# cyberlife-coder/velesdb

Hardware: AMD Instinct MI355X
Metric: qps_at_recall10_1Mx768_k10 (higher is better)
Workload: dtype f32; 1 GPU; 1000000x768 f32 cosine, k=10, exact distance sweep + fused GPU top-k (BASELINE configs[1]); 1024 queries/step, 1024 queries per corpus pass (sweep_topk_gemm_bf16_pp<dot, WIDE> over normalised bf16 images of rows and queries (cosine; ping-po; rows=1000000, dim=768, k=10, parallelism=replicas x1 (query stream split, no collective)

## Files before the change

velesdb_amd/csrc/sweep_wide.hip:

```cpp
#include <algorithm>

#include "vdb_device.hpp"
#include "vdb_kernels.hpp"
#include "vdb_wide.hpp"
#include "vdb_block_select.hpp"

namespace vdb {

__device__ __forceinline__ float wide_eps(uint32_t dim, const float* rho_q, const uint32_t* rho_max_bits, uint32_t q, float extra = 0.0f) {
  const float acc = 16.0f * (float)dim * 5.9604645e-8f;
  if (!rho_q || !rho_max_bits) return 2.0f * 3.90625e-3f * 1.002f + 1.6e-5f + acc + extra;
  const float rm = __uint_as_float(*rho_max_bits), rq = rho_q[q];
  return (rm + rq + 3.0f * rm * rq) * 1.002f + acc + 4e-6f + extra;
}

__device__ __forceinline__ uint64_t wide_tau_key(float s_k, float delta, bool* ok, float extra = 0.0f) {
  const float lowered = s_k - 2.0f * delta * 1.01f - extra - fabsf(s_k) * 1e-6f;
  *ok = lowered == lowered && fabsf(lowered) < 3.0e38f;
  return make_key<true>(lowered, 0u);
}
__device__ __forceinline__ uint64_t wide_tau_closed() { return make_key<true>(3.0e38f, 0u); }

template <int METRIC>
__global__ __launch_bounds__(256) void wide_seed_kernel(WideArgs a, const uint64_t* seed_keys, uint32_t ngrp) {
  __shared__ uint32_t hist[256];
  __shared__ uint32_t ctl[2];
  const uint32_t q = blockIdx.x, tid = threadIdx.x;
  constexpr int NPT = kWideSeedGroups / 256;
  uint64_t keys[NPT];
  uint32_t mine = 0;
#pragma unroll
  for (int j = 0; j < NPT; j++) {
    const uint32_t i = tid + 256u * (uint32_t)j;
    keys[j] = i < ngrp ? seed_keys[(size_t)q * ngrp + i] : kKeyInvalid;
    mine += keys[j] != kKeyInvalid ? 1u : 0u;
  }
  const float eps = wide_eps(a.dim, a.rho_q, a.rho_max_bits, q, a.eps_extra);
  const float d = METRIC == kCosine ? eps * 1.001f + 4e-7f : eps * 1.001f * a.qnorms[q] * __uint_as_float(*a.norm_max_bits) + 1e-30f;
  __shared__ uint32_t total;
  if (tid == 0) total = 0;
  __syncthreads();
  if (mine) atomicAdd(&total, mine);
  __syncthreads();
  const uint32_t valid = total;
  bool ok = valid >= a.k && d == d;
  uint64_t tau = wide_tau_closed();
  if (ok) {
    __shared__ uint64_t s256[256];
    const uint32_t hi = ngrp <= 256 ? block_kth_hi_256(keys[0], a.k, s256, ctl) : block_kth_hi<NPT>(keys, a.k, hist, ctl);
    tau = wide_tau_key(key_score<true>((uint64_t)hi << 32), d, &ok);
    if (!ok) tau = wide_tau_closed();
  }
  if (tid == 0) {
    a.delta[q] = d;
    a.tau[q] = tau;
    a.cnt[q] = 0;
    a.state[q] = ok ? 0u : kWideGivenUp;
  }
}

template <int NPT>
__device__ int wide_next_tau(const WideArgs& a, uint32_t raw, const uint64_t (&keys)[NPT], float delta, float extra, uint64_t old, uint32_t* hist,
                             uint32_t* ctl, uint64_t* s256, uint64_t* tau_out) {
  if (raw > a.cap) return 2;
  if (raw < a.k) return 0;
  const uint32_t hi = raw <= 256 ? block_kth_hi_256(keys[0], a.k, s256, ctl, (raw + 7u) & ~7u) : block_kth_hi<NPT>(keys, a.k, hist, ctl);
  bool ok;
  uint64_t tau = wide_tau_key(key_score<true>((uint64_t)hi << 32), delta, &ok, extra);
  if (!ok) return 2;
  if (tau > old) tau = old;
  *tau_out = tau;
  return 1;
}

__global__ __launch_bounds__(256) void wide_reseed_kernel(WideArgs a) {
  __shared__ uint32_t hist[256];
  __shared__ uint32_t ctl[2];
  __shared__ uint32_t wsum[4];
  __shared__ uint64_t s256[256];
  const uint32_t q = blockIdx.x, tid = threadIdx.x;
  const uint32_t state = a.state[q], raw = a.cnt[q];
  const float delta = a.delta[q], extra = a.extra ? a.extra[q] : 0.0f;
  const uint64_t old = a.tau[q];
  if (state & kWideGivenUp) return;
  constexpr int NPT = kWideCap / 256;
  uint64_t* list = a.keys + (size_t)q * a.cap;
  uint64_t keys[NPT];
  keys[0] = list[tid];
  if (tid >= raw) keys[0] = kKeyInvalid;
#pragma unroll
  for (int j = 1; j < NPT; j++) {
    const uint32_t i = tid + 256u * (uint32_t)j;
    keys[j] = (i < raw && i < a.cap) ? list[i] : kKeyInvalid;
  }
  uint64_t tau = 0;
  const int what = wide_next_tau<NPT>(a, raw, keys, delta, extra, old, hist, ctl, s256, &tau);
  if (what == 0) return;
  if (what == 2) {
    if (tid == 0) {
      a.state[q] |= kWideGivenUp;
      a.tau[q] = wide_tau_closed();
    }
    return;
  }
  uint32_t keep = 0;
#pragma unroll
  for (int j = 0; j < NPT; j++) keep += (keys[j] != kKeyInvalid && keys[j] < tau) ? 1u : 0u;
  uint32_t incl = keep;
  const uint32_t lane = tid & 63u, w = tid >> 6;
#pragma unroll
  for (int o = 1; o < 64; o <<= 1) {
    const uint32_t up = __shfl_up(incl, o, 64);
    if ((int)lane >= o) incl += up;
  }
  if (lane == 63) wsum[w] = incl;
  __syncthreads();
  uint32_t base = incl - keep;
  for (uint32_t x = 0; x < w; x++) base += wsum[x];
#pragma unroll
  for (int j = 0; j < NPT; j++)
    if (keys[j] != kKeyInvalid && keys[j] < tau) list[base++] = keys[j];
  if (tid == 0) {
    a.cnt[q] = wsum[0] + wsum[1] + wsum[2] + wsum[3];
    a.tau[q] = tau;
  }
}

template <int METRIC>
__global__ __launch_bounds__(256) void wide_rerank_verify(WideArgs a, WideOutArgs o, bool fuse) {
  extern __shared__ __attribute__((aligned(16))) unsigned char smem[];
  constexpr uint32_t kStep = 64, kStride = kStep + 4, kChunk = 64;
  float* qs = reinterpret_cast<float*>(smem);
  uint64_t* ekeys = reinterpret_cast<uint64_t*>(qs + o.dim_pad);
  float* stage = reinterpret_cast<float*>(ekeys + kWidePoolMax);
  uint32_t* crow = reinterpret_cast<uint32_t*>(stage + 2 * kChunk * kStride);
  uint64_t* kth = reinterpret_cast<uint64_t*>(crow + kChunk);
  __shared__ uint32_t cand[kWidePoolMax];
  __shared__ uint32_t hist[256];
  __shared__ uint32_t ctl[2];
  __shared__ uint32_t wsum[4];
  __shared__ uint64_t s256[256];
  const uint32_t tid = threadIdx.x, qi = blockIdx.x;
  auto stamp = [&](int i) {
    if (o.stamps && tid == 0) o.stamps[(size_t)qi * 8 + i] = wall_clock64();
  };
  stamp(0);
  const float* q = o.queries + (size_t)qi * o.q_stride;
  const uint64_t* list = a.keys + (size_t)qi * a.cap;
  float qreg[4];
#pragma unroll
  for (int j = 0; j < 4; j++) {
    const uint32_t i = tid + 256u * (uint32_t)j;
    qreg[j] = i < a.dim ? q[i] : 0.0f;
  }
  const uint64_t first = list[tid];
  const float qn = METRIC == kCosine ? a.qnorms[qi] : 0.0f;
  const uint32_t raw = a.cnt[qi];
  bool given_up = (a.state[qi] & kWideGivenUp) != 0 || raw > a.cap;
  uint64_t tau_fin = a.tau[qi];
  const float delta = a.delta[qi], extra = a.extra ? a.extra[qi] : 0.0f;
  uint32_t n = 0;
  if (fuse) {
    constexpr int NPT = kWideCap / 256;
    uint64_t keys[NPT];
    keys[0] = (!given_up && tid < raw) ? first : kKeyInvalid;
#pragma unroll
    for (int j = 1; j < NPT; j++) {
      const uint32_t i = tid + 256u * (uint32_t)j;
      keys[j] = (!given_up && i < raw) ? list[i] : kKeyInvalid;
    }
    if (!given_up) {
      uint64_t t = 0;
      const int what = wide_next_tau<NPT>(a, raw, keys, delta, extra, tau_fin, hist, ctl, s256, &t);
      if (what == 2) given_up = true;
      if (what == 1) tau_fin = t;
    }
    uint32_t keep = 0;
#pragma unroll
    for (int j = 0; j < NPT; j++) keep += (keys[j] != kKeyInvalid && keys[j] < tau_fin) ? 1u : 0u;
    uint32_t incl = keep;
    const uint32_t lane = tid & 63u, w = tid >> 6;
#pragma unroll
    for (int s = 1; s < 64; s <<= 1) {
      const uint32_t up = __shfl_up(incl, s, 64);
      if ((int)lane >= s) incl += up;
    }
    if (lane == 63) wsum[w] = incl;
    __syncthreads();
    uint32_t base = incl - keep;
    for (uint32_t x = 0; x < w; x++) base += wsum[x];
    const uint32_t total = wsum[0] + wsum[1] + wsum[2] + wsum[3];
    if (total > kWidePoolMax) given_up = true;
    if (!given_up) {
      n = total;
#pragma unroll
      for (int j = 0; j < NPT; j++)
        if (keys[j] != kKeyInvalid && keys[j] < tau_fin) cand[base++] = key_row(keys[j]);
    }
  } else {
    if (raw > kWidePoolMax) given_up = true;
    n = given_up ? 0u : raw;
    if (tid < n) cand[tid] = key_row(first);
    for (uint32_t i = tid + 256; i < n; i += 256) cand[i] = key_row(list[i]);
  }
  stamp(1);
#pragma unroll
  for (int j = 0; j < 4; j++) {
    const uint32_t i = tid + 256u * (uint32_t)j;
    if (i < o.dim_pad) qs[i] = qreg[j];
  }
  for (uint32_t i = tid + 1024; i < o.dim_pad; i += 256) qs[i] = i < a.dim ? q[i] : 0.0f;
  if (tid == 0) *kth = kKeyInvalid;
  for (uint32_t c0 = 0; c0 < n; c0 += kChunk) {
    const uint32_t nc = min(kChunk, n - c0);
    __syncthreads();
    if (tid < nc) crow[tid] = cand[c0 + tid];
    __syncthreads();
    uint32_t sh = 0;
    while (sh < 3 && (nc << (sh + 1)) <= kChunk) sh++;
    const uint32_t W = kStep << sh, rowf4 = (kStep / 4) << sh, wstride = W + 4;
    const uint32_t nf4 = nc * rowf4;
    float4 vr[4][4];
    auto fetch = [&](float4 (&v)[4], uint32_t U) {
#pragma unroll
      for (int i = 0; i < 4; i++) {
        const uint32_t f = tid + 256u * (uint32_t)i;
        const uint32_t r = f >> (4 + sh), c4 = f & (rowf4 - 1);
        v[i] = (f < nf4 && U + 4 * c4 < a.dim) ? ld4(o.rows + (size_t)crow[r] * o.row_stride + U + 4 * c4) : make_float4(0.0f, 0.0f, 0.0f, 0.0f);
      }
    };
    auto park = [&](const float4 (&v)[4], uint32_t buf) {
#pragma unroll
      for (int i = 0; i < 4; i++) {
        const uint32_t f = tid + 256u * (uint32_t)i;
        const uint32_t r = f >> (4 + sh), c4 = f & (rowf4 - 1);
        if (f < nf4) *reinterpret_cast<float4*>(stage + (size_t)buf * kChunk * kStride + (size_t)r * wstride + 4 * c4) = v[i];
      }
    };
    float acc = 0.0f;
    auto chain = [&](uint32_t U, uint32_t buf) {
      if (tid < nc) {
        const float* x = stage + (size_t)buf * kChunk * kStride + (size_t)tid * wstride;
        const uint32_t groups = min(W, o.dim_pad - U) / 16;
#pragma unroll 4
        for (uint32_t m = 0; m < groups; m++) {
          float xr[16];
#pragma unroll
          for (int e = 0; e < 16; e += 4) {
            const float4 w = *reinterpret_cast<const float4*>(x + 16 * m + e);
            xr[e] = w.x; xr[e + 1] = w.y; xr[e + 2] = w.z; xr[e + 3] = w.w;
          }
          const uint32_t base = U + 16 * m;
#pragma unroll
          for (int c = 0; c < 4; c++)
#pragma unroll
            for (int kk = 0; kk < 4; kk++) acc = __builtin_fmaf(xr[4 * kk + c], qs[base + 4 * kk + c], acc);
        }
      }
    };
    const uint32_t nsteps = (o.dim_pad + W - 1) / W;
    fetch(vr[0], 0);
    if (1 < nsteps) fetch(vr[1], W);
    if (2 < nsteps) fetch(vr[2], 2 * W);
    const float vnorm = (METRIC == kCosine && tid < nc) ? o.norms[crow[tid]] : 1.0f;
    park(vr[0], 0);
    __syncthreads();
    if (c0 == 0) stamp(2);
    for (uint32_t s0 = 0; s0 < nsteps; s0 += 4) {
#pragma unroll
      for (int j = 0; j < 4; j++) {
        const uint32_t st = s0 + (uint32_t)j;
        if (st < nsteps) {
          if (st + 3 < nsteps) fetch(vr[(j + 3) & 3], (st + 3) * W);
          chain(st * W, st & 1u);
          if (st + 1 < nsteps) park(vr[(j + 1) & 3], (st + 1) & 1u);
          __syncthreads();
        }
      }
    }
    if (c0 == 0) stamp(3);
    if (tid < nc) {
      const uint32_t row = crow[tid];
      const float score = finish_score<METRIC>(acc, qn, vnorm);
      ekeys[c0 + tid] = make_key<true>(score, row);
    }
  }
  __syncthreads();
  stamp(4);
  const uint32_t kk = min(a.k, n);
  for (uint32_t i = tid; i < n; i += 256) {
    const uint64_t key = ekeys[i];
    uint32_t rank = 0;
    for (uint32_t j = 0; j < n; j++) rank += ekeys[j] < key ? 1u : 0u;
    if (rank < kk) {
      const uint32_t row = key_row(key);
      o.out_ids[(size_t)qi * a.k + rank] = o.ext_ids ? o.ext_ids[row] : (uint64_t)row;
      o.out_scores[(size_t)qi * a.k + rank] = key_score<true>(key);
      if (rank + 1 == a.k) *kth = key;
    }
  }
  for (uint32_t e = kk + tid; e < a.k; e += 256) {
    o.out_ids[(size_t)qi * a.k + e] = ~0ull;
    o.out_scores[(size_t)qi * a.k + e] = __uint_as_float(0x7FC00000u);
  }
  __syncthreads();
  stamp(5);
  if (tid == 0) {
    bool ok = !given_up && n >= a.k;
    if (ok) {
      const float A = key_score<true>(tau_fin);
      const double Ek = (double)key_score<true>(*kth);
      ok = Ek > (double)A + (double)delta;
    }
    if (fuse) a.tau[qi] = tau_fin;
    o.flags[qi] = ok ? 0u : 1u;
    if (!ok) {
      const uint32_t j = atomicAdd(o.qcount, 1u);
      o.qmap[j] = qi;
      o.qslot[qi] = j;
    }
    o.out_n[qi] = kk;
    if (o.stamps) {
      o.stamps[(size_t)qi * 8 + 6] = wall_clock64();
      o.stamps[(size_t)qi * 8 + 7] = ((unsigned long long)raw << 32) | n;
    }
  }
}

__global__ __launch_bounds__(256) void wide_seed_l2_kernel(WideArgs a, const uint64_t* seed_keys, uint32_t ngrp, uint32_t dim_a) {
  __shared__ uint32_t hist[256];
  __shared__ uint32_t ctl[2];
  __shared__ uint32_t total;
  const uint32_t q = blockIdx.x, tid = threadIdx.x;
  constexpr int NPT = kWideSeedGroups / 256;
  uint64_t keys[NPT];
  uint32_t mine = 0;
#pragma unroll
  for (int j = 0; j < NPT; j++) {
    const uint32_t i = tid + 256u * (uint32_t)j;
    keys[j] = i < ngrp ? seed_keys[(size_t)q * ngrp + i] : kKeyInvalid;
    mine += keys[j] != kKeyInvalid ? 1u : 0u;
  }
  if (tid == 0) total = 0;
  __syncthreads();
  if (mine) atomicAdd(&total, mine);
  __syncthreads();
  const uint32_t valid = total;
  const float nmax = __uint_as_float(*a.norm_max_bits), hmax = 0.5f * nmax * nmax, qn = a.qnorms[q];
  const float acc = 16.0f * (float)dim_a * 5.9604645e-8f;
  float eps_r = 2.0f * 3.90625e-3f * 1.002f + 1.6e-5f + acc;
  if (a.rho_q && a.rho_max_bits) {
    const float rm = __uint_as_float(*a.rho_max_bits), rq = a.rho_q[q];
    eps_r = (rm + rq + 3.0f * rm * rq) * 1.002f + acc;
  }
  const float d = eps_r * 1.001f * qn * nmax + (1.6e-5f + acc) * hmax + 1e-30f;
  const float slack = 8.0f * (float)a.dim * 5.9604645e-8f * (qn * qn + nmax * nmax) * 1.01f + 1e-30f;
  bool ok = valid >= a.k && d == d && slack == slack;
  uint64_t tau = wide_tau_closed();
  if (ok) {
    const uint32_t hi = block_kth_hi<NPT>(keys, a.k, hist, ctl);
    tau = wide_tau_key(key_score<true>((uint64_t)hi << 32), d, &ok, slack);
    if (!ok) tau = wide_tau_closed();
  }
  if (tid == 0) {
    a.delta[q] = d;
    a.extra[q] = slack;
    a.tau[q] = tau;
    a.cnt[q] = 0;
    a.state[q] = ok ? 0u : kWideGivenUp;
  }
}

__global__ __launch_bounds__(256) void wide_rerank_l2(WideArgs a, WideOutArgs o) {
  __shared__ uint64_t ekeys[kWidePoolMax];
  __shared__ float esums[kWidePoolMax];
  __shared__ float kth_sum;
  const int lane = lane_id();
  const uint32_t wib = threadIdx.x >> 6, tid = threadIdx.x, qi = blockIdx.x;
  const uint32_t raw = a.cnt[qi];
  const bool given_up = (a.state[qi] & kWideGivenUp) != 0 || raw > kWidePoolMax || raw > a.cap;
  const uint32_t n = given_up ? 0u : raw;
  const float* q = o.queries + (size_t)qi * o.q_stride;
  const uint64_t* list = a.keys + (size_t)qi * a.cap;
  const int d4 = (int)((a.dim + 3) / 4);
  if (tid == 0) kth_sum = __uint_as_float(0x7FC00000u);
  for (uint32_t c0 = wib; c0 < n; c0 += 16) {
    const float* p[4];
    uint32_t rowv[4];
    float acc[4] = {0.0f, 0.0f, 0.0f, 0.0f};
#pragma unroll
    for (int u = 0; u < 4; u++) {
      const uint32_t c = min(c0 + 4u * (uint32_t)u, n - 1u);
      rowv[u] = key_row(list[c]);
      p[u] = o.rows + (size_t)rowv[u] * o.row_stride;
    }
    for (int ch = lane; ch < d4; ch += 64) {
      const int nv = (int)a.dim - ch * 4;
      float4 x[4];
#pragma unroll
      for (int u = 0; u < 4; u++) x[u] = ld4(p[u] + ch * 4);
      float4 qq;
      if (nv >= 4) {
        qq = make_float4(q[ch * 4], q[ch * 4 + 1], q[ch * 4 + 2], q[ch * 4 + 3]);
#pragma unroll
        for (int u = 0; u < 4; u++) acc[u] = chain4<kOpL2>(acc[u], qq, x[u]);
      } else {
        qq = make_float4(q[ch * 4], nv > 1 ? q[ch * 4 + 1] : 0.f, nv > 2 ? q[ch * 4 + 2] : 0.f, 0.f);
#pragma unroll
        for (int u = 0; u < 4; u++) acc[u] = chain4_tail<kOpL2>(acc[u], qq, x[u], nv);
      }
    }
#pragma unroll
    for (int u = 0; u < 4; u++) {
      const uint32_t c = c0 + 4u * (uint32_t)u;
      const float sum = butterfly_all(acc[u]);
      if (lane == 0 && c < n) {
        esums[c] = sum;
        ekeys[c] = make_key<false>(finish_score<kEuclidean>(sum, 0.f, 0.f), rowv[u]);
      }
    }
  }
  __syncthreads();
  const uint32_t kk = min(a.k, n);
  for (uint32_t i = tid; i < n; i += 256) {
    const uint64_t key = ekeys[i];
    uint32_t rank = 0;
    for (uint32_t j = 0; j < n; j++) rank += ekeys[j] < key ? 1u : 0u;
    if (rank < kk) {
      const uint32_t row = key_row(key);
      o.out_ids[(size_t)qi * a.k + rank] = o.ext_ids ? o.ext_ids[row] : (uint64_t)row;
      o.out_scores[(size_t)qi * a.k + rank] = key_score<false>(key);
      if (rank + 1 == a.k) kth_sum = esums[i];
    }
  }
  for (uint32_t e = kk + tid; e < a.k; e += 256) {
    o.out_ids[(size_t)qi * a.k + e] = ~0ull;
    o.out_scores[(size_t)qi * a.k + e] = __uint_as_float(0x7FC00000u);
  }
  __syncthreads();
  if (tid == 0) {
    bool ok = !given_up && n >= a.k;
    if (ok) {
      const double A = (double)key_score<true>(a.tau[qi]);
      const double qn = (double)a.qnorms[qi];
      const double Ek = (double)kth_sum;
      ok = (Ek + (double)a.extra[qi] + 1e-6 * Ek) < qn * qn - 2.0 * (A + (double)a.delta[qi]);
    }
    o.flags[qi] = ok ? 0u : 1u;
    if (!ok) {
      const uint32_t j = atomicAdd(o.qcount, 1u);
      o.qmap[j] = qi;
      o.qslot[qi] = j;
    }
    o.out_n[qi] = kk;
  }
}

template <int METRIC>
__global__ __launch_bounds__(256) void wide_rerank_sq8(WideArgs a, WideOutArgs o) {
  extern __shared__ __attribute__((aligned(16))) unsigned char smem[];
  float* qs = reinterpret_cast<float*>(smem);
  uint64_t* ekeys = reinterpret_cast<uint64_t*>(qs + ((a.dim + 3) & ~3u));
  float* qred = reinterpret_cast<float*>(ekeys + kWidePoolMax);
  uint64_t* kth = reinterpret_cast<uint64_t*>(qred + 2);
  const uint32_t tid = threadIdx.x, qi = blockIdx.x;
  const uint32_t raw = a.cnt[qi];
  const bool given_up = (a.state[qi] & kWideGivenUp) != 0 || raw > kWidePoolMax || raw > a.cap;
  const uint32_t n = given_up ? 0u : raw;
  const float* q = o.queries + (size_t)qi * o.q_stride;
  for (uint32_t i = tid; i < a.dim; i += 256) qs[i] = q[i];
  if (tid == 0) *kth = kKeyInvalid;
  __syncthreads();
  if (tid == 64) {
    float s1 = 0.0f;
    for (uint32_t d = 0; d < a.dim; d++) s1 = __fadd_rn(s1, qs[d]);
    qred[0] = s1;
  }
  if (tid == 128) {
    float s2 = 0.0f;
    for (uint32_t d = 0; d < a.dim; d++) s2 = __fadd_rn(s2, __fmul_rn(qs[d], qs[d]));
    qred[1] = s2;
  }
  __syncthreads();
  const uint64_t* list = a.keys + (size_t)qi * a.cap;
  for (uint32_t c = tid; c < n; c += 256) {
    const uint32_t row = key_row(list[c]);
    const float mn = o.sq8_min[row], range = __fsub_rn(o.sq8_max[row], mn);
    const uint32_t* cw = reinterpret_cast<const uint32_t*>(o.sq8_codes + (size_t)row * o.sq8_stride);
    float acc = 0.0f;
    if (range < 1.1920929e-07f) {
      acc = __fmul_rn(qred[0], mn);
    } else {
      const float scale = __fdiv_rn(range, 255.0f);
      for (uint32_t i = 0; i < a.dim; i += 4) {
        const uint32_t w = cw[i >> 2];
#pragma unroll
        for (int e = 0; e < 4; e++)
          if (i + e < a.dim) {
            const float dq = __fadd_rn(__fmul_rn((float)((w >> (8 * e)) & 0xFFu), scale), mn);
            acc = __fadd_rn(acc, __fmul_rn(qs[i + e], dq));
          }
      }
    }
    float score = acc;
    if (METRIC == kCosine) {
      const float denom = sqrtf(__fmul_rn(qred[1], o.sq8_nsq[row]));
      score = denom < 1.1920929e-07f ? 0.0f : __fdiv_rn(acc, denom);
    }
    ekeys[c] = make_key<true>(score, row);
  }
  __syncthreads();
  const uint32_t kk = min(a.k, n);
  for (uint32_t i = tid; i < n; i += 256) {
    const uint64_t key = ekeys[i];
    uint32_t rank = 0;
    for (uint32_t j = 0; j < n; j++) rank += ekeys[j] < key ? 1u : 0u;
    if (rank < kk) {
      const uint32_t row = key_row(key);
      o.out_ids[(size_t)qi * a.k + rank] = o.ext_ids ? o.ext_ids[row] : (uint64_t)row;
      o.out_scores[(size_t)qi * a.k + rank] = key_score<true>(key);
      if (rank + 1 == a.k) *kth = key;
    }
  }
  for (uint32_t e = kk + tid; e < a.k; e += 256) {
    o.out_ids[(size_t)qi * a.k + e] = ~0ull;
    o.out_scores[(size_t)qi * a.k + e] = __uint_as_float(0x7FC00000u);
  }
  __syncthreads();
  if (tid == 0) {
    bool ok = !given_up && n >= a.k;
    if (ok) {
      const float A = key_score<true>(a.tau[qi]);
      const double Ek = (double)key_score<true>(*kth);
      ok = Ek > (double)A + (double)a.delta[qi];
    }
    o.flags[qi] = ok ? 0u : 1u;
    if (!ok) {
      const uint32_t j = atomicAdd(o.qcount, 1u);
      o.qmap[j] = qi;
      o.qslot[qi] = j;
    }
    o.out_n[qi] = kk;
  }
}

void launch_wide_seed(int metric, const WideArgs& a, const uint64_t* seed_keys, uint32_t ngrp, uint32_t nq, hipStream_t st) {
  if (metric == kCosine)
    hipLaunchKernelGGL((wide_seed_kernel<kCosine>), dim3(nq), dim3(256), 0, st, a, seed_keys, ngrp);
  else
    hipLaunchKernelGGL((wide_seed_kernel<kDot>), dim3(nq), dim3(256), 0, st, a, seed_keys, ngrp);
}
void launch_wide_reseed(const WideArgs& a, uint32_t nq, hipStream_t st) { hipLaunchKernelGGL(wide_reseed_kernel, dim3(nq), dim3(256), 0, st, a); }
void launch_wide_seed_l2(const WideArgs& a, const uint64_t* seed_keys, uint32_t ngrp, uint32_t dim_a, uint32_t nq, hipStream_t st) {
  hipLaunchKernelGGL(wide_seed_l2_kernel, dim3(nq), dim3(256), 0, st, a, seed_keys, ngrp, dim_a);
}
void launch_wide_rerank_l2(const WideArgs& a, const WideOutArgs& o, uint32_t nq, hipStream_t st) {
  hipLaunchKernelGGL(wide_rerank_l2, dim3(nq), dim3(256), 0, st, a, o);
}
void launch_wide_rerank_sq8(int metric, const WideArgs& a, const WideOutArgs& o, uint32_t nq, hipStream_t st) {
  const size_t lds = ((size_t)((a.dim + 3) & ~3u) * 4 + (size_t)kWidePoolMax * 8 + 8 + 8 + 15) & ~(size_t)15;
  if (metric == kCosine)
    hipLaunchKernelGGL((wide_rerank_sq8<kCosine>), dim3(nq), dim3(256), lds, st, a, o);
  else
    hipLaunchKernelGGL((wide_rerank_sq8<kDot>), dim3(nq), dim3(256), lds, st, a, o);
}
size_t wide_rerank_lds_bytes(uint32_t dim_pad) {
  return ((size_t)dim_pad * 4 + (size_t)kWidePoolMax * 8 + 2 * (size_t)64 * 68 * 4 + 64 * 4 + 8 + 15) & ~(size_t)15;
}
void launch_wide_rerank(int metric, const WideArgs& a, const WideOutArgs& o, uint32_t nq, bool fuse_final_reseed, hipStream_t st) {
  const size_t lds = wide_rerank_lds_bytes(o.dim_pad);
  if (metric == kCosine)
    hipLaunchKernelGGL((wide_rerank_verify<kCosine>), dim3(nq), dim3(256), lds, st, a, o, fuse_final_reseed);
  else
    hipLaunchKernelGGL((wide_rerank_verify<kDot>), dim3(nq), dim3(256), lds, st, a, o, fuse_final_reseed);
}

}
```

Before: 788,800 queries/s.

## Alias rerank LDS regions by phase and read query via scalar loads

Rewrites the rerank-verify kernel's shared-memory plan so candidate ids, exact keys, the staging buffer and selection scratch alias each other by phase. This shrinks LDS, and launch bounds now request 4 blocks per SIMD. The query vector stays in LDS only when it fits next to the candidate pool; otherwise it is read through constant-address-space (scalar) loads in a hand-scheduled, double-buffered FMA loop. Staging rows drop padding and use an XOR swizzle against bank conflicts, and per-query scalars are made wave-uniform with readfirstlane. This risks aliasing hazards between phases (cand is interleaved inside ekeys) and adds complexity, all to raise occupancy and cut LDS traffic in the rerank stage.

```diff
diff --git a/velesdb_amd/csrc/sweep_wide.hip b/velesdb_amd/csrc/sweep_wide.hip
--- a/velesdb_amd/csrc/sweep_wide.hip
+++ b/velesdb_amd/csrc/sweep_wide.hip
@@ -3,6 +3,7 @@
 #include "vdb_device.hpp"
 #include "vdb_kernels.hpp"
 #include "vdb_wide.hpp"
+#include "vdb_wide_rerank_plan.hpp"
 #include "vdb_block_select.hpp"
 
 namespace vdb {
@@ -126,39 +127,45 @@
   }
 }
 
+typedef const __attribute__((address_space(4))) float* wide_cfloat_ptr;
+
 template <int METRIC>
-__global__ __launch_bounds__(256) void wide_rerank_verify(WideArgs a, WideOutArgs o, bool fuse) {
+__global__ __launch_bounds__(256, 4) void wide_rerank_verify(WideArgs a, WideOutArgs o, bool fuse) {
   extern __shared__ __attribute__((aligned(16))) unsigned char smem[];
-  constexpr uint32_t kStep = 64, kStride = kStep + 4, kChunk = 64;
-  float* qs = reinterpret_cast<float*>(smem);
-  uint64_t* ekeys = reinterpret_cast<uint64_t*>(qs + o.dim_pad);
-  float* stage = reinterpret_cast<float*>(ekeys + kWidePoolMax);
-  uint32_t* crow = reinterpret_cast<uint32_t*>(stage + 2 * kChunk * kStride);
-  uint64_t* kth = reinterpret_cast<uint64_t*>(crow + kChunk);
-  __shared__ uint32_t cand[kWidePoolMax];
-  __shared__ uint32_t hist[256];
-  __shared__ uint32_t ctl[2];
-  __shared__ uint32_t wsum[4];
-  __shared__ uint64_t s256[256];
+  constexpr uint32_t kStep = kWideRerankStep, kChunk = kWideRerankChunk, kBuf = kWideRerankBufFloats;
+  static_assert(kWideRerankPool == kWidePoolMax, "vdb_wide_rerank_plan.hpp restates it");
+  const WideRerankPlan lp = wide_rerank_plan(o.dim_pad, a.k);
+  uint64_t* ekeys = reinterpret_cast<uint64_t*>(smem + lp.ekeys.off);
+  uint32_t* cand = reinterpret_cast<uint32_t*>(ekeys);
+  float* stage = reinterpret_cast<float*>(smem + lp.stage.off);
+  uint64_t* s256 = reinterpret_cast<uint64_t*>(smem + lp.s256.off);
+  uint32_t* hist = reinterpret_cast<uint32_t*>(smem + lp.hist.off);
+  uint32_t* ctl = reinterpret_cast<uint32_t*>(smem + lp.ctl.off);
+  uint32_t* wsum = reinterpret_cast<uint32_t*>(smem + lp.wsum.off);
+  uint64_t* kth = reinterpret_cast<uint64_t*>(smem + lp.kth.off);
   const uint32_t tid = threadIdx.x, qi = blockIdx.x;
   auto stamp = [&](int i) {
     if (o.stamps && tid == 0) o.stamps[(size_t)qi * 8 + i] = wall_clock64();
   };
   stamp(0);
   const float* q = o.queries + (size_t)qi * o.q_stride;
-  const uint64_t* list = a.keys + (size_t)qi * a.cap;
   float qreg[4];
 #pragma unroll
   for (int j = 0; j < 4; j++) {
     const uint32_t i = tid + 256u * (uint32_t)j;
     qreg[j] = i < a.dim ? q[i] : 0.0f;
   }
+  const wide_cfloat_ptr qc = (wide_cfloat_ptr)q;
+  const uint64_t* list = a.keys + (size_t)qi * a.cap;
   const uint64_t first = list[tid];
-  const float qn = METRIC == kCosine ? a.qnorms[qi] : 0.0f;
-  const uint32_t raw = a.cnt[qi];
-  bool given_up = (a.state[qi] & kWideGivenUp) != 0 || raw > a.cap;
-  uint64_t tau_fin = a.tau[qi];
-  const float delta = a.delta[qi], extra = a.extra ? a.extra[qi] : 0.0f;
+  auto uni = [](uint32_t v) { return (uint32_t)__builtin_amdgcn_readfirstlane((int)v); };
+  auto unif = [&](float v) { return __uint_as_float(uni(__float_as_uint(v))); };
+  auto uni64 = [&](uint64_t v) { return ((uint64_t)uni((uint32_t)(v >> 32)) << 32) | uni((uint32_t)v); };
+  const float qn = METRIC == kCosine ? unif(a.qnorms[qi]) : 0.0f;
+  const uint32_t raw = uni(a.cnt[qi]);
+  bool given_up = (uni(a.state[qi]) & kWideGivenUp) != 0 || raw > a.cap;
+  uint64_t tau_fin = uni64(a.tau[qi]);
+  const float delta = unif(a.delta[qi]), extra = a.extra ? unif(a.extra[qi]) : 0.0f;
   uint32_t n = 0;
   if (fuse) {
     constexpr int NPT = kWideCap / 256;
@@ -195,38 +202,44 @@
       n = total;
 #pragma unroll
       for (int j = 0; j < NPT; j++)
-        if (keys[j] != kKeyInvalid && keys[j] < tau_fin) cand[base++] = key_row(keys[j]);
+        if (keys[j] != kKeyInvalid && keys[j] < tau_fin) cand[2 * base++] = key_row(keys[j]);
     }
   } else {
     if (raw > kWidePoolMax) given_up = true;
     n = given_up ? 0u : raw;
-    if (tid < n) cand[tid] = key_row(first);
-    for (uint32_t i = tid + 256; i < n; i += 256) cand[i] = key_row(list[i]);
-  }
+    if (tid < n) cand[2 * tid] = key_row(first);
+    for (uint32_t i = tid + 256; i < n; i += 256) cand[2 * i] = key_row(list[i]);
+  }
+  n = uni(n);
+  tau_fin = uni64(tau_fin);
+  given_up = uni(given_up ? 1u : 0u) != 0;
   stamp(1);
-#pragma unroll
-  for (int j = 0; j < 4; j++) {
-    const uint32_t i = tid + 256u * (uint32_t)j;
-    if (i < o.dim_pad) qs[i] = qreg[j];
-  }
-  for (uint32_t i = tid + 1024; i < o.dim_pad; i += 256) qs[i] = i < a.dim ? q[i] : 0.0f;
-  if (tid == 0) *kth = kKeyInvalid;
+  const bool q_lds = wide_rerank_query_in_lds(o.dim_pad, n);
+  const float* qs = reinterpret_cast<const float*>(smem + lp.ekeys.off + wide_rerank_query_off(o.dim_pad));
+  if (q_lds) {
+    float* qw = const_cast<float*>(qs);
+#pragma unroll
+    for (int j = 0; j < 4; j++) {
+      const uint32_t i = tid + 256u * (uint32_t)j;
+      if (i < o.dim_pad) qw[i] = qreg[j];
+    }
+    for (uint32_t i = tid + 1024; i < o.dim_pad; i += 256) qw[i] = i < a.dim ? q[i] : 0.0f;
+  }
+  __syncthreads();
   for (uint32_t c0 = 0; c0 < n; c0 += kChunk) {
     const uint32_t nc = min(kChunk, n - c0);
-    __syncthreads();
-    if (tid < nc) crow[tid] = cand[c0 + tid];
-    __syncthreads();
+    const uint32_t* crow = cand + 2 * c0;
     uint32_t sh = 0;
     while (sh < 3 && (nc << (sh + 1)) <= kChunk) sh++;
-    const uint32_t W = kStep << sh, rowf4 = (kStep / 4) << sh, wstride = W + 4;
+    const uint32_t W = kStep << sh, rowf4 = (kStep / 4) << sh;
     const uint32_t nf4 = nc * rowf4;
     float4 vr[4][4];
-    auto fetch = [&](float4 (&v)[4], uint32_t U) {
+    auto fetch = [&](float4 (&v)[4], uint32_t U, bool on) {
 #pragma unroll
       for (int i = 0; i < 4; i++) {
         const uint32_t f = tid + 256u * (uint32_t)i;
         const uint32_t r = f >> (4 + sh), c4 = f & (rowf4 - 1);
-        v[i] = (f < nf4 && U + 4 * c4 < a.dim) ? ld4(o.rows + (size_t)crow[r] * o.row_stride + U + 4 * c4) : make_float4(0.0f, 0.0f, 0.0f, 0.0f);
+        v[i] = (on && f < nf4 && U + 4 * c4 < a.dim) ? ld4(o.rows + (size_t)crow[2 * r] * o.row_stride + U + 4 * c4) : make_float4(0.0f, 0.0f, 0.0f, 0.0f);
       }
     };
     auto park = [&](const float4 (&v)[4], uint32_t buf) {
@@ -234,35 +247,85 @@
       for (int i = 0; i < 4; i++) {
         const uint32_t f = tid + 256u * (uint32_t)i;
         const uint32_t r = f >> (4 + sh), c4 = f & (rowf4 - 1);
-        if (f < nf4) *reinterpret_cast<float4*>(stage + (size_t)buf * kChunk * kStride + (size_t)r * wstride + 4 * c4) = v[i];
+        if (f < nf4) *reinterpret_cast<float4*>(stage + (size_t)buf * kBuf + (size_t)r * W + 4 * (c4 ^ (r & (rowf4 - 1)))) = v[i];
       }
     };
     float acc = 0.0f;
-    auto chain = [&](uint32_t U, uint32_t buf) {
+    auto load_x = [&](float4 (&x)[4], const float* xrow, uint32_t sw, uint32_t m) {
+#pragma unroll
+      for (int e = 0; e < 4; e++) x[e] = *reinterpret_cast<const float4*>(xrow + 4 * ((4 * m + (uint32_t)e) ^ sw));
+    };
+    auto load_q = [&](float (&qv)[16], uint32_t base) {
+      const wide_cfloat_ptr p = qc + base;
+#pragma unroll
+      for (int e = 0; e < 16; e++) qv[e] = p[e];
+    };
+    auto load_q_tail = [&](float (&qv)[16], uint32_t base) {
+      const wide_cfloat_ptr p = qc + base;
+#pragma unroll
+      for (int e = 0; e < 16; e++) qv[e] = base + e < a.dim ? p[e] : 0.0f;
+    };
+    auto fma16 = [&](const float4 (&x)[4], const float (&qv)[16]) {
+      const float xr[16] = {x[0].x, x[0].y, x[0].z, x[0].w, x[1].x, x[1].y, x[1].z, x[1].w,
+                            x[2].x, x[2].y, x[2].z, x[2].w, x[3].x, x[3].y, x[3].z, x[3].w};
+#pragma unroll
+      for (int c = 0; c < 4; c++)
+#pragma unroll
+        for (int kk = 0; kk < 4; kk++) acc = __builtin_fmaf(xr[4 * kk + c], qv[4 * kk + c], acc);
+    };
+    auto chain = [&](uint32_t U_v, uint32_t buf) {
       if (tid < nc) {
-        const float* x = stage + (size_t)buf * kChunk * kStride + (size_t)tid * wstride;
-        const uint32_t groups = min(W, o.dim_pad - U) / 16;
-#pragma unroll 4
-        for (uint32_t m = 0; m < groups; m++) {
-          float xr[16];
-#pragma unroll
-          for (int e = 0; e < 16; e += 4) {
-            const float4 w = *reinterpret_cast<const float4*>(x + 16 * m + e);
-            xr[e] = w.x; xr[e + 1] = w.y; xr[e + 2] = w.z; xr[e + 3] = w.w;
+        const uint32_t U = (uint32_t)__builtin_amdgcn_readfirstlane((int)U_v);
+        const float* xrow = stage + (size_t)buf * kBuf + (size_t)tid * W;
+        const uint32_t sw = tid & (rowf4 - 1);
+        const uint32_t groups = (uint32_t)__builtin_amdgcn_readfirstlane((int)(min(W, o.dim_pad - U) / 16));
+        float4 xa[4], xb[4];
+        float qa[16], qb[16];
+        if (q_lds) {
+#pragma unroll 2
+          for (uint32_t m = 0; m < groups; m++) {
+            load_x(xa, xrow, sw, m);
+#pragma unroll
+            for (int e = 0; e < 4; e++) {
+              const float4 w = *reinterpret_cast<const float4*>(qs + U + 16 * m + 4 * e);
+              qa[4 * e] = w.x; qa[4 * e + 1] = w.y; qa[4 * e + 2] = w.z; qa[4 * e + 3] = w.w;
+            }
+            fma16(xa, qa);
           }
-          const uint32_t base = U + 16 * m;
-#pragma unroll
-          for (int c = 0; c < 4; c++)
-#pragma unroll
-            for (int kk = 0; kk < 4; kk++) acc = __builtin_fmaf(xr[4 * kk + c], qs[base + 4 * kk + c], acc);
+        } else if (U + 16 * groups <= a.dim) {
+          load_x(xa, xrow, sw, 0);
+          load_q(qa, U);
+#pragma unroll 1
+          for (uint32_t m = 0; m < groups; m += 2) {
+            __builtin_amdgcn_s_waitcnt(0xC07F);
+            __builtin_amdgcn_sched_barrier(0);
+            load_x(xb, xrow, sw, m + 1);
+            load_q(qb, U + 16 * (m + 1));
+            __builtin_amdgcn_sched_barrier(0);
+            fma16(xa, qa);
+            __builtin_amdgcn_s_waitcnt(0xC07F);
+            __builtin_amdgcn_sched_barrier(0);
+            const uint32_t m2 = min(m + 2, groups - 2);
+            load_x(xa, xrow, sw, m2);
+            load_q(qa, U + 16 * m2);
+            __builtin_amdgcn_sched_barrier(0);
+            fma16(xb, qb);
+          }
+        } else {
+#pragma unroll 1
+          for (uint32_t m = 0; m < groups; m++) {
+            load_x(xa, xrow, sw, m);
+            load_q_tail(qa, U + 16 * m);
+            fma16(xa, qa);
+          }
         }
       }
     };
     const uint32_t nsteps = (o.dim_pad + W - 1) / W;
-    fetch(vr[0], 0);
-    if (1 < nsteps) fetch(vr[1], W);
-    if (2 < nsteps) fetch(vr[2], 2 * W);
-    const float vnorm = (METRIC == kCosine && tid < nc) ? o.norms[crow[tid]] : 1.0f;
+    fetch(vr[0], 0, true);
+    fetch(vr[1], W, 1 < nsteps);
+    fetch(vr[2], 2 * W, 2 < nsteps);
+    const float vnorm = (METRIC == kCosine && tid < nc) ? o.norms[crow[2 * tid]] : 1.0f;
     park(vr[0], 0);
     __syncthreads();
     if (c0 == 0) stamp(2);
@@ -271,7 +334,7 @@
       for (int j = 0; j < 4; j++) {
         const uint32_t st = s0 + (uint32_t)j;
         if (st < nsteps) {
-          if (st + 3 < nsteps) fetch(vr[(j + 3) & 3], (st + 3) * W);
+          fetch(vr[(j + 3) & 3], (st + 3) * W, st + 3 < nsteps);
           chain(st * W, st & 1u);
           if (st + 1 < nsteps) park(vr[(j + 1) & 3], (st + 1) & 1u);
           __syncthreads();
@@ -280,11 +343,12 @@
     }
     if (c0 == 0) stamp(3);
     if (tid < nc) {
-      const uint32_t row = crow[tid];
+      const uint32_t row = crow[2 * tid];
       const float score = finish_score<METRIC>(acc, qn, vnorm);
       ekeys[c0 + tid] = make_key<true>(score, row);
     }
   }
+  if (tid == 0) *kth = kKeyInvalid;
   __syncthreads();
   stamp(4);
   const uint32_t kk = min(a.k, n);
@@ -564,11 +628,8 @@
   else
     hipLaunchKernelGGL((wide_rerank_sq8<kDot>), dim3(nq), dim3(256), lds, st, a, o);
 }
-size_t wide_rerank_lds_bytes(uint32_t dim_pad) {
-  return ((size_t)dim_pad * 4 + (size_t)kWidePoolMax * 8 + 2 * (size_t)64 * 68 * 4 + 64 * 4 + 8 + 15) & ~(size_t)15;
-}
 void launch_wide_rerank(int metric, const WideArgs& a, const WideOutArgs& o, uint32_t nq, bool fuse_final_reseed, hipStream_t st) {
-  const size_t lds = wide_rerank_lds_bytes(o.dim_pad);
+  const size_t lds = wide_rerank_plan(o.dim_pad, a.k).bytes;
   if (metric == kCosine)
     hipLaunchKernelGGL((wide_rerank_verify<kCosine>), dim3(nq), dim3(256), lds, st, a, o, fuse_final_reseed);
   else
diff --git a/velesdb_amd/csrc/vdb_wide_rerank_plan.hpp b/velesdb_amd/csrc/vdb_wide_rerank_plan.hpp
--- /dev/null
+++ b/velesdb_amd/csrc/vdb_wide_rerank_plan.hpp
@@ -0,0 +1,39 @@
+#pragma once
+#include <stdint.h>
+
+namespace vdb {
+
+constexpr uint32_t kWideRerankPool = 1024;
+constexpr uint32_t kWideRerankChunk = 64;
+constexpr uint32_t kWideRerankStep = 64;
+constexpr uint32_t kWideRerankBufFloats = kWideRerankChunk * kWideRerankStep;
+constexpr uint32_t kWideRerankLdsBudget = 40960;
+
+struct WideRerankRegion {
+  uint32_t off, bytes;
+  uint32_t first_phase, last_phase;
+};
+struct WideRerankPlan {
+  WideRerankRegion ekeys, stage, s256, hist, ctl, wsum, kth;
+  uint32_t bytes;
+};
+
+constexpr WideRerankPlan wide_rerank_plan(uint32_t dim_pad, uint32_t k) {
+  (void)dim_pad;
+  (void)k;
+  WideRerankPlan p{};
+  p.ekeys = {0, kWideRerankPool * 8, 1, 3};
+  p.stage = {p.ekeys.off + p.ekeys.bytes, 2 * kWideRerankBufFloats * 4, 2, 2};
+  p.s256 = {p.stage.off, 256 * 8, 1, 1};
+  p.hist = {p.s256.off + p.s256.bytes, 256 * 4, 1, 1};
+  p.ctl = {p.hist.off + p.hist.bytes, 2 * 4, 1, 1};
+  p.wsum = {p.ctl.off + p.ctl.bytes, 4 * 4, 1, 1};
+  p.kth = {p.stage.off, 8, 3, 3};
+  p.bytes = (p.stage.off + p.stage.bytes + 15u) & ~15u;
+  return p;
+}
+
+constexpr bool wide_rerank_query_in_lds(uint32_t dim_pad, uint32_t n) { return (uint64_t)n * 8 + (uint64_t)dim_pad * 4 <= (uint64_t)kWideRerankPool * 8; }
+constexpr uint32_t wide_rerank_query_off(uint32_t dim_pad) { return kWideRerankPool * 8 - dim_pad * 4; }
+
+}
```

After: 791,900 queries/s (median of 6 runs). Within noise of the previous version (+0.4%).
